# kfirc1503/generative-audio

Hardware: AMD Instinct MI355X
Metric: spectrogram-frames/sec, NPPC K=5 FullSubNet+ train step (higher is better)
Workload: dtype bf16

## Files before the change

### generative-audio_amd/csrc/tcn.hip

```cpp
#include <cstdlib>
#include "common.h"
#include "mfma_tile.h"
#include "nppc_hip.h"

namespace {


template <typename T, int EPI>
__global__ __launch_bounds__(256) void gemm_nt_kernel(GemmArgs g) {
  const int ks = g.ksplit > 1 ? g.ksplit : 1;
  const int z = blockIdx.z / ks, ksl = blockIdx.z % ks;
  const T* A = reinterpret_cast<const T*>(g.A) + (size_t)z * g.strideA + (size_t)ksl * g.K;
  const T* B = reinterpret_cast<const T*>(g.B) + (size_t)z * g.strideB + (size_t)ksl * g.K;
  const int lane = threadIdx.x & 63, wave = threadIdx.x >> 6, n = lane & 15, q = lane >> 4;
  const int r0 = blockIdx.x * 128 + wave * 32, c0 = blockIdx.y * 64;
  const T* ap = A + (size_t)(r0 + n) * g.lda + 8 * q;
  const T* bp = B + (size_t)(c0 + n) * g.ldb + 8 * q;
  f32x4 acc[2][4];
  nt_reg_mainloop<T>(acc, g.K / 32, g.lda, g.ldb, [&](int kk) { return ap + 32 * kk; }, [&](int kk) { return bp + 32 * kk; },
                     g.relu_in);

  const NtEpilogue<T, EPI> ep(g, z, blockIdx.x * 128);
  float s1 = 0.f, s2 = 0.f;
#pragma unroll
// ... 929 lines not shown
                     lda, (const bf16_t*)B1, ldb1, nt1, (const bf16_t*)B2, ldb2, N2, C, ldc, (long)M * ldc, R / ksplit, rowsum);
  NPPC_CHECK_LAUNCH();
  return NPPC_OK;
}

extern "C" int nppc_gemm_tn_splitk_batched(const void* A, long lda, long sA, const void* B, long ldb, long sB, float* C, long ldc,
                                           long sC, int M, int N, long R, int ksplit, int batch, void* stream) {
  if (batch < 1) return NPPC_EBADARG;
  return launch_tn(A, lda, B, ldb, C, ldc, M, N, R, ksplit, 1, 0, 0, stream, batch, sA, sB, sC);
}

extern "C" int nppc_gemm_tn_splitk_taps(const void* A, long lda, const void* B, long ldb, float* C, long ldc, int M, int N,
                                        long R, int ksplit, int Wp, int shift_a, void* stream) {
  return launch_tn(A, lda, B, ldb, C, ldc, M, N, R, ksplit, 9, Wp, shift_a, stream);
}
```

### generative-audio_amd/csrc/train_ops.hip

```cpp
#include "common.h"
#include "nppc_hip.h"

namespace {

template <typename T>
__global__ __launch_bounds__(256) void transpose_kernel(const T* __restrict__ in, T* __restrict__ out, int rows, int cols,
                                                        long ld_in, long ld_out, long sIn, long sOut, int relu) {
  __shared__ float tile[32][33];
  in += (size_t)blockIdx.z * sIn;
  out += (size_t)blockIdx.z * sOut;
  const int r0 = blockIdx.x * 32, c0 = blockIdx.y * 32;
  const int tx = threadIdx.x & 31, ty = threadIdx.x >> 5;
  for (int i = ty; i < 32; i += 8) {
    const int r = r0 + i, c = c0 + tx;
    float v = 0.f;
    if (r < rows && c < cols) v = to_f32<T>(in[(size_t)r * ld_in + c]);
    if (relu) v = fmaxf(v, 0.f);
    tile[i][tx] = v;
  }
  __syncthreads();
  for (int i = ty; i < 32; i += 8) {
    const int c = c0 + i, r = r0 + tx;
    if (c < cols && r < rows) out[(size_t)c * ld_out + r] = from_f32<T>(tile[tx][i]);
  }
// ... 326 lines not shown
  dst += (size_t)blockIdx.z * sDst;
  __shared__ float tile[32][33];
  const int c0 = blockIdx.x * 32, r0 = blockIdx.y * 32;
  const int tx = threadIdx.x & 31, ty = threadIdx.x >> 5;
  for (int i = ty; i < 32; i += 8) {
    const int c = c0 + i, r = r0 + tx;
    float a = 0.f;
    if (c < ncols && r < rows)
      for (int s = 0; s < S; ++s) a += slabs[(size_t)s * slab_stride + (size_t)c * ld + r];
    tile[i][tx] = a;
  }
  __syncthreads();
  for (int i = ty; i < 32; i += 8) {
    const int r = r0 + i, c = c0 + tx;
    if (r < rows && c < ncols) dst[(size_t)r * dst_ld + c] = tile[tx][i];
  }
}

__global__ void adam_kernel(float* __restrict__ p, const float* __restrict__ g, float* __restrict__ m, float* __restrict__ v,
                            long n, float lr, float b1, float b2, float eps, float wd, float bc1, float bc2_sqrt,
                            float gscale, const double* __restrict__ sumsq, float max_norm,
                            const unsigned* const* __restrict__ guards = nullptr, int n_guards = 0, float* poison = nullptr) {
  for (int i = 0; i < n_guards; ++i)
    if (*guards[i] != 0u) {
      if (poison && blockIdx.x == 0 && threadIdx.x == 0) *poison = __builtin_nanf("");
      return;
    }
  if (sumsq) {
    const float total = (float)sqrt(sumsq[0]) * gscale;
    const float coef = max_norm / (total + 1e-6f);
// ... 183 lines not shown
  hipLaunchKernelGGL(reduce_slabs_kernel, dim3(gx, 1, batch), dim3(256), 0, (hipStream_t)stream, slabs, S, slab_stride, ld,
                     dst, dst_ld, rows, col0, ncols, permH, accumulate, sSlab, sDst);
  NPPC_CHECK_LAUNCH();
  return NPPC_OK;
}

int nppc_reduce_slabs_t(const float* slabs, int S, long slab_stride, long ld, float* dst, long dst_ld, int rows, int ncols,
                        long sSlab, long sDst, int batch, void* stream) {
  if (!slabs || !dst || S < 1 || rows <= 0 || ncols <= 0 || batch < 1) return NPPC_EBADARG;
  hipLaunchKernelGGL(reduce_slabs_t_kernel, dim3(ceil_div(ncols, 32), ceil_div(rows, 32), batch), dim3(256), 0,
                     (hipStream_t)stream, slabs, S, slab_stride, ld, dst, dst_ld, rows, ncols, sSlab, sDst);
  NPPC_CHECK_LAUNCH();
  return NPPC_OK;
}

int nppc_adam_step(float* p, const float* g, float* m, float* v, long n, double lr, double b1, double b2, double eps,
                   double wd, int step, double gscale, void* stream) {
  if (!p || !g || !m || !v || n <= 0 || step < 1) return NPPC_EBADARG;
  const double bc1 = 1.0 - pow(b1, (double)step);
  const double bc2s = sqrt(1.0 - pow(b2, (double)step));
  const int grid = (int)((n + 255) / 256 > 2048 ? 2048 : (n + 255) / 256);
  hipLaunchKernelGGL(adam_kernel, dim3(grid), dim3(256), 0, (hipStream_t)stream, p, g, m, v, n, (float)lr, (float)b1, (float)b2,
                     (float)eps, (float)wd, (float)bc1, (float)bc2s, (float)gscale, (const double*)nullptr, 0.f);
  NPPC_CHECK_LAUNCH();
  return NPPC_OK;
}

int nppc_adam_step_guarded(float* p, const float* g, float* m, float* v, long n, double lr, double b1, double b2, double eps,
                           double wd, int step, double gscale, const void* guards, int n_guards, float* poison, void* stream) {
  if (!p || !g || !m || !v || n <= 0 || step < 1 || n_guards < 0 || (n_guards > 0 && !guards)) return NPPC_EBADARG;
// ... 24 lines not shown
```

### generative-audio_amd/nppc_audio/_hip.py

```python
import ctypes
import os
import threading

import torch

_HERE = os.path.dirname(os.path.abspath(__file__))
LIB_PATH = os.path.join(_HERE, "libnppc_hip.so")

PREC_BF16 = 0
PREC_F32 = 1
_ERR = {1: "bad argument", 2: "kernel launch failed", 3: "unsupported shape/configuration"}

_lib = None

c_p = ctypes.c_void_p
c_i = ctypes.c_int
c_l = ctypes.c_long
c_f = ctypes.c_float


def lib():
    global _lib
    if _lib is None:
        if not os.path.exists(LIB_PATH):
# ... 23 lines not shown
def check(rc, what):
    if rc != 0:
        raise RuntimeError(f"{what} failed: {_ERR.get(rc, rc)}")


def ptr_array(tensors):
    for t in tensors:
        assert t.is_cuda and t.is_contiguous()
    return (ctypes.c_void_p * len(tensors))(*[t.data_ptr() for t in tensors])


def mid_bwd_part_elems(B, C, Tp, batch):
    n = c_l()
    call("nppc_tcn_mid_bwd_part_elems", B, C, Tp, batch, ctypes.byref(n))
    return n.value


def conv_thin_part_elems():
    n = c_l()
    call("nppc_conv_thin_part_elems", ctypes.byref(n))
    return n.value


def masked_mse_work_elems():
    n = c_l()
    call("nppc_masked_mse_work_elems", ctypes.byref(n))
    return n.value


def crm_mse_work_elems():
# ... 51 lines not shown
                           I, I, I, I, I, I, P],
    "nppc_scale_transpose": [I, P, P, P, I, I, I, I, I, I, P],
    "nppc_gemm_nt": [I, I, P, L, L, P, L, L, P, L, L, P, L, P, L, L, P, L, P, L, I, I, I, I, I, I, I, I, I, P],
    "nppc_tcn_mid_bwd_part_elems": [I, I, I, I, PL],
    "nppc_tcn_mid_bwd": [I, P, P, P, P, P, P, P, P, P, P, P, P, P, P, P, P, P, P, P, P, P, P, P, P, P, P, I, I, I, P,
                         I, I, I, I, I, F, L, L, L, I, I, P],
    "nppc_tcn_mid_bwd_finish": [P, L, P, L, I, I, I, P, P, P, P, P, P, P, P, P, P, I, I, L, L, I, I, P],
    "nppc_gemm_nt_colsum": [I, I, P, L, L, P, L, L, P, L, L, P, L, P, L, L, I, I, I, I, I, I, I, P, P],
    "nppc_gemm_nt_gn": [I, P, L, L, P, L, L, P, L, L, P, P, L, P, L, L, P, L, D, F, I, I, I, I, I, I, I, P],
    "nppc_tcn_pack_sconv": [I, P, P, P, P, P, P, P, I, I, I, I, I, I, L, L, L, L, P],
    "nppc_gemm_nt_splitk": [I, P, L, P, L, P, L, I, I, L, I, P],
    "nppc_gemm_tn_splitk": [P, L, P, L, P, L, I, I, L, I, P],
    "nppc_gemm_tn_splitk_rowsum": [P, L, P, L, P, L, I, I, L, I, P, P],
    "nppc_gemm_tn_splitk2": [P, L, P, L, I, P, L, I, P, L, I, L, I, P, P],
    "nppc_gemm_tn_splitk_batched": [P, L, L, P, L, L, P, L, L, I, I, L, I, I, P],
    "nppc_reduce_slabs_t": [P, I, L, L, P, L, I, I, L, L, I, P],
    "nppc_gemm_tn_splitk_taps": [P, L, P, L, P, L, I, I, L, I, I, I, P],
    "nppc_tcn_dwconv": [I, P, P, P, P, P, P, P, P, P, I, I, I, I, I, I, F, L, L, L, I, P],
    "nppc_tcn_gn_apply": [I, P, P, P, P, P, I, I, I, I, I, F, L, L, L, I, P],
    "nppc_pack_matrix": [I, P, P, I, I, I, I, I, P],
    "nppc_pack_matrix_batched": [I, P, P, I, I, I, I, I, I, I, L, L, L, L, P],
    "nppc_subband_mean": [I, P, I, P, I, L, P, P, P, I, I, I, I, I, P],
    "nppc_subband_stage": [I, P, I, P, I, L, P, P, I, I, I, I, I, I, I, I, P],
    "nppc_sb_head": [I, P, P, P, P, L, I, I, I, I, I, P],
    "nppc_gram": [P, P, P, P, P, I, I, L, P],
    "nppc_combine": [P, P, P, P, P, P, P, I, I, L, P],
    "nppc_gs_solve": [P, P, P, I, I, I, P],
    "nppc_gs_bwd_solve": [P, P, P, P, I, I, I, P],
    "nppc_loss_solve": [P, P, P, P, P, P, P, P, P, P, I, I, P],
    "nppc_loss_bwd_coef": [P, P, P, F, F, P, I, I, P],
    "nppc_loss_bwd_coef_dev": [P, P, P, P, F, F, P, I, I, P],
    "nppc_transpose": [I, P, P, I, I, L, L, L, L, I, I, P],
    "nppc_colsum": [I, P, P, I, I, L, L, L, I, P, L, P],
    "nppc_colsum_scratch_elems": [I, I, I, PL],
    "nppc_sb_head_bwd": [I, P, P, P, P, P, P, L, I, I, I, I, I, P],
    "nppc_subband_stage_bwd": [I, P, P, P, P, P, P, I, I, I, I, I, L, I, I, I, P],
    "nppc_subband_unfold_bwd": [I, P, P, P, P, P, I, I, I, I, I, I, I, I, P],
    "nppc_reduce_slabs": [P, I, L, L, P, L, I, I, I, I, I, L, L, I, P],
    "nppc_adam_step": [P, P, P, P, L, D, D, D, D, D, I, D, P],
    "nppc_adam_step_guarded": [P, P, P, P, L, D, D, D, D, D, I, D, P, I, P, P],
    "nppc_loss_solve_eps": [P, P, P, P, P, P, P, P, P, P, I, I, D, I, P],
    "nppc_loss_solve_obj": [P, P, P, P, P, P, P, P, P, P, I, I, D, I, F, P, P],
    "nppc_mix_snr": [P, P, P, F, P, P, P, I, I, P],
    "nppc_inpaint_prepare": [P, P, P, I, F, P, P, P, I, I, I, I, I, P],
    "nppc_time_to_spec_mask": [P, P, I, I, I, I, I, I, P],
    "nppc_stft_pair": [P, P, P, P, I, I, I, I, P],
    "nppc_dropout": [I, P, L, L, I, F, L, I, P, P],
    "nppc_pca_work_elems": [I, I, I, PL],
    "nppc_pca_batch": [P, I, I, I, I, P, P, P, P, P, P, P],
    "nppc_pair_loss": [P, P, P, P, P, P, P, P, P, I, I, L, D, P],
    "nppc_pair_loss_bwd": [P, P, P, P, F, F, P, I, I, L, P],
    "nppc_metric_rows": [P, P, P, P, P, L, P],
    "nppc_rows_gram": [P, I, P, I, L, P, P],
# ... 153 lines not shown
```

### generative-audio_amd/nppc_audio/engine.py

```python
import ctypes

import numpy as np
import torch

from . import _hip as H
from .ops_lstm import (PackedLSTM, PackedLSTMBwd, ROW_PAD, WGRAD_SPLITS, bwd_head_fusable, forward_x_ld, lstm2_backward, lstm2_forward,
                       own_workspaces, padded_rows,
                       rows_view, workspace)

TCN_HIDDEN = 512
TCN_DILATIONS = (1, 2, 5, 9, 1, 2, 5, 9)
BRANCHES = ("", "_real", "_imag")
EPI_PLAIN, EPI_PRELU_STATS, EPI_RESIDUAL, EPI_RELU, EPI_PLAIN_F32, EPI_MASK_POS = 0, 1, 2, 3, 4, 5


def rup(a, b):
    return (a + b - 1) // b * b


TCN_WGRAD_SPLITS = 8
TCN_WGRAD_MAIN_BLOCKS = 1


class FlatParams:

    def __init__(self, module, device):
        named = list(module.named_parameters())
        total = sum(p.numel() for _, p in named)
        self.flat = torch.empty(total, dtype=torch.float32, device=device)
        self.grad = None
        self.off = {}
        o = 0
        for n, p in named:
            k = p.numel()
            self.flat[o:o + k].copy_(p.detach().reshape(-1))
            p.data = self.flat[o:o + k].view(p.shape)
# ... 371 lines not shown
                self.g(dest[3]).copy_(self.g(dest[2]))

        if self.prec == H.PREC_BF16 and K4 % 128 == 0 and Hd % 64 == 0 and KX % 64 == 0:
            S = WGRAD_SPLITS
            assert 64 * S <= ROW_PAD
            slab = ws("slab", (S * K4 * max(Hd, KX),), torch.float32)
            fold_bias = K4 % 256 == 0 and Hd % 128 == 0 and (K4 // 256) * (Hd // 128) * S >= 256
            if (guards is not None and fold_bias and Hd % 192 == 0 and KX == 64 and Tv > 1
                    and (K4 // 256) * (Hd // 192 + 1) * S >= 256):
                h1_guard, h2_guard = guards
                rows = (Rr + 64 * S - 1) // (64 * S) * (64 * S)
                slab = ws("slab2", (S * K4 * 2 * Hd,), torch.float32)
                rsum = ws("rowsum", (S, K4), torch.float32)
                H.call("nppc_gemm_tn_splitk2", dg1, K4, h1_guard, Hd, Hd, x_rows, KX, KX, slab, Hd + KX, K4, rows, S, None, s)
                n1 = K4 * (Hd + KX)
                H.call("nppc_reduce_slabs", slab, S, n1, Hd + KX, self.g(q + "weight_hh_l0"), Hd, K4, 0, Hd, Hd, 0, 0, 0, 1, s)
                H.call("nppc_reduce_slabs", slab, S, n1, Hd + KX, self.g(q + "weight_ih_l0"), I, K4, Hd, I, Hd, 0, 0, 0, 1, s)
                H.call("nppc_reduce_slabs", slab, S, n1, Hd + KX, self.g(q + "bias_ih_l0"), 1, K4, Hd + I, 1, Hd, 0, 0, 0, 1, s)
                self.g(q + "bias_hh_l0").copy_(self.g(q + "bias_ih_l0"))
                H.call("nppc_gemm_tn_splitk2", dg2, K4, h1_rows, Hd, Hd, h2_guard, Hd, Hd, slab, 2 * Hd, K4, rows, S, rsum, s)
                n2 = K4 * 2 * Hd
                H.call("nppc_reduce_slabs", slab, S, n2, 2 * Hd, self.g(q + "weight_ih_l1"), Hd, K4, 0, Hd, Hd, 0, 0, 0, 1, s)
                H.call("nppc_reduce_slabs", slab, S, n2, 2 * Hd, self.g(q + "weight_hh_l1"), Hd, K4, Hd, Hd, Hd, 0, 0, 0, 1, s)
                H.call("nppc_reduce_slabs", rsum, S, K4, 1, self.g(q + "bias_ih_l1"), 1, K4, 0, 1, Hd, 0, 0, 0, 1, s)
                self.g(q + "bias_hh_l1").copy_(self.g(q + "bias_ih_l1"))
                jobs = []
            for dg, off, inp, width, dest in jobs:
                rows = (Rr - off + 64 * S - 1) // (64 * S) * (64 * S)
                if fold_bias and dest[0] == "bias":
                    continue
                if fold_bias and dest == ("w", q + "weight_ih_l1"):
                    rsum = ws("rowsum", (S, K4), torch.float32)
                    H.call("nppc_gemm_tn_splitk_rowsum", dg.view(-1)[off * K4:], K4, inp, width, slab, width, K4, width, rows, S,
                           rsum, s)
                    H.call("nppc_reduce_slabs", rsum, S, K4, 1, self.g(q + "bias_ih_l1"), 1, K4, 0, 1, Hd, 0, 0, 0, 1, s)
                    self.g(q + "bias_hh_l1").copy_(self.g(q + "bias_ih_l1"))
                else:
                    H.call("nppc_gemm_tn_splitk", dg.view(-1)[off * K4:], K4, inp, width, slab, width, K4, width, rows, S, s)
                scatter(slab, S, K4, width, dest)
            if head is not None:
# ... 125 lines not shown
        h1b = ws("h1b", (3, B, Tp, TCN_HIDDEN))
        h2b = ws("h2b", (3, B, Tp, TCN_HIDDEN))
        Smid = ws("Smid", (3, B, TCN_HIDDEN // 64, 8), torch.float64)
        n_part = H.mid_bwd_part_elems(B, TCN_HIDDEN, Tp, 3)
        Pmid = ws("Pmid", (8, n_part), torch.float32)
        lay = self.fp.off["fb_model.sequence_model.1.conv1x1.weight"][0] - self.fp.off["fb_model.sequence_model.0.conv1x1.weight"][0]

        def finish_mid(lo, hi):
            pre_ = f"fb_model.sequence_model.{lo}."
            H.call("nppc_tcn_mid_bwd_finish", Pmid[lo], n_part, cpL[lo] if cs_ok else None, 3 * (R // 128) * ldC, R // 128, ldC, C,
                   self.g(pre_ + "norm2.weight"), self.g(pre_ + "norm2.bias"), self.g(pre_ + "norm1.weight"), self.g(pre_ + "norm1.bias"),
                   self.g(pre_ + "depthwise_conv.weight"), self.g(pre_ + "depthwise_conv.bias"), self.g(pre_ + "prelu1.weight"),
                   self.g(pre_ + "prelu2.weight"), self.g(pre_ + "conv1x1.bias"), self.g(pre_ + "sconv.bias") if cs_ok else None,
                   B, TCN_HIDDEN, sP, lay, 3, hi - lo, s)
        early = self.grad_range_hook is not None and self.early_buckets_ok
        dXo, dXi = dXa, dXb
        for i in range(7, -1, -1):
            pre = f"fb_model.sequence_model.{i}."
            dil = TCN_DILATIONS[i]
            st1, st2 = d["stats"][i, 0], d["stats"][i, 1]
            y1, y2, Xin = d["y1"][i], d["y2"][i], d["X"][i]
            if tn_ok:
                dXo, dXi, a2, h2b = dXL[i + 1], dXL[i], a2L[i], h2L[i]
            else:
                a2 = d["a2"]
            if not cs_ok:
                H.colsum(prec, dXo, self.g(pre + "sconv.bias"), R, C, ldC, R * ldC, sP, 3,
                         lambda n: ws("cs_sconv", (n,), torch.float32), s)
            H.call("nppc_gemm_nt", prec, EPI_PLAIN, dXo, ldC, R * ldC, self.W2T[i], ldC, TCN_HIDDEN * ldC, h1b, TCN_HIDDEN,
                   sAct, None, 0, None, 0, 0, None, 0, None, 0, R, TCN_HIDDEN, ldC, Tp, Tv, TCN_HIDDEN, 0, 3, 1, s)
            H.call("nppc_tcn_mid_bwd", prec, h1b, y2, y1, st1, st2, Smid, Pmid[i], self.p(pre + "norm1.weight"), self.p(pre + "norm1.bias"),
                   self.p(pre + "norm2.weight"), self.p(pre + "norm2.bias"), self.p(pre + "depthwise_conv.weight"),
                   self.p(pre + "prelu1.weight"), self.p(pre + "prelu2.weight"), a2, h2b, self.g(pre + "norm2.weight"),
                   self.g(pre + "norm2.bias"), self.g(pre + "norm1.weight"), self.g(pre + "norm1.bias"),
                   self.g(pre + "depthwise_conv.weight"), self.g(pre + "depthwise_conv.bias"), self.g(pre + "prelu1.weight"),
                   self.g(pre + "prelu2.weight"), self.g(pre + "conv1x1.bias"),
                   cpL[i] if cs_ok else None, R // 128, ldC, C, self.g(pre + "sconv.bias") if cs_ok else None,
                   B, TCN_HIDDEN, Tp, Tv, dil, 1e-8, sAct, B * 2, sP, 3, 0, s)
            if i == 4 and early:
                finish_mid(4, 8)
            if tn_ok:
                inline = i < TCN_WGRAD_MAIN_BLOCKS
                wslab = ws("slab_main", (3 * S2 * TCN_HIDDEN * ldC,), torch.float32) if inline else slab2

                def sconv_wgrad(a2=a2, dXo=dXo, dest=self.g(pre + "sconv.weight"), wslab=wslab):
                    q = H.stream()
                    H.call("nppc_gemm_tn_splitk_batched", a2, TCN_HIDDEN, sAct, dXo, ldC, R * ldC, wslab, ldC,
                           S2 * TCN_HIDDEN * ldC, TCN_HIDDEN, ldC, R, S2, 3, q)
                    H.call("nppc_reduce_slabs_t", wslab, S2, TCN_HIDDEN * ldC, ldC, dest, TCN_HIDDEN, C, TCN_HIDDEN,
                           S2 * TCN_HIDDEN * ldC, sP, 3, q)
                if inline:
                    sconv_wgrad()
                else:
                    on_side(sconv_wgrad)
            else:
                H.call("nppc_transpose", prec, dXo, tA, R, ldC, ldC, R, R * ldC, sTA, 0, 3, s)
                H.call("nppc_transpose", prec, a2, tB, R, TCN_HIDDEN, TCN_HIDDEN, R, sAct, sTB, 0, 3, s)
                self._wgrad(tA, R, sTA, tB, R, sTB, Cr, TCN_HIDDEN, R, S2, pre + "sconv.weight", TCN_HIDDEN, C, TCN_HIDDEN,
                            slab2, batch=3, sDst=sP)
            if tn_ok:
                def c1_wgrad(h2b=h2b, Xin=Xin, dest=self.g(pre + "conv1x1.weight"), wslab=wslab):
                    q = H.stream()
                    H.call("nppc_gemm_tn_splitk_batched", h2b, TCN_HIDDEN, sAct, Xin, ldC, R * ldC, wslab, ldC,
                           S2 * TCN_HIDDEN * ldC, TCN_HIDDEN, ldC, R, S2, 3, q)
                    H.call("nppc_reduce_slabs", wslab, S2, TCN_HIDDEN * ldC, ldC, dest, C, TCN_HIDDEN, 0, C, 0, 0,
                           S2 * TCN_HIDDEN * ldC, sP, 3, q)
                if inline:
                    c1_wgrad()
                else:
                    on_side(c1_wgrad)
            else:
                H.call("nppc_transpose", prec, h2b, tA, R, TCN_HIDDEN, TCN_HIDDEN, R, sAct, sTA, 0, 3, s)
                H.call("nppc_transpose", prec, Xin, tB, R, ldC, ldC, R, R * ldC, sTB, 0, 3, s)
                self._wgrad(tA, R, sTA, tB, R, sTB, TCN_HIDDEN, ldC, R, S2, pre + "conv1x1.weight", C, TCN_HIDDEN, C, slab2,
                            batch=3, sDst=sP)
# ... 10 lines not shown
                        a = self.fp.off[f"fb_model{br}.sequence_model.4.conv1x1.weight"][0]
                        b, shp = self.fp.off[f"fb_model{br}.sequence_model.7.sconv.bias"]
                        self.grad_range_hook(G, a, b + int(np.prod(shp)))
                on_side(blocks_done)
        finish_mid(0, 4 if early else 8)
        if tn_ok:
            dXo = dXL[0]
        if self.nm == 1:
            H.call("nppc_subband_unfold_bwd", prec, dx, d["sbscale"], Dsb, self.mult, dXo[0], ldC, B, F, Tp, Tv, self.nb, self.G,
                   self.KX, s)
        sv = d["tsse_saved"]
        n_ws = ctypes.c_long()
        H.call("nppc_tsse_bwd_ws_elems", 3 * self.nm, B, F, self.ks[0], self.ks[1], self.ks[2], ctypes.byref(n_ws))
        dsg = ws("dsg", (n_ws.value,), torch.float32)
        att = "channel_attention."
        H.call("nppc_tsse_bwd_maps", prec, dXo, R * ldC, H.ptr_array(d["maps"]), 3 * self.nm, d["rs"],
               self.p(att + "smallConv1d.0.weight"), self.p(att + "middleConv1d.0.weight"), self.p(att + "largeConv1d.0.weight"),
               self.ks[0], self.ks[1], self.ks[2], self.p(att + "feature_concate_fc.weight"), self.p(att + "fc1.weight"),
               self.p(att + "fc2.weight"), self.sAtt, sv["ns"], sv["pre"], sv["sq"], sv["h1"], sv["sg"], dsg,
               self.g(att + "smallConv1d.0.weight"), self.g(att + "smallConv1d.0.bias"),
               self.g(att + "middleConv1d.0.weight"), self.g(att + "middleConv1d.0.bias"),
               self.g(att + "largeConv1d.0.weight"), self.g(att + "largeConv1d.0.bias"),
               self.g(att + "feature_concate_fc.weight"), self.g(att + "feature_concate_fc.bias"),
               self.g(att + "fc1.weight"), self.g(att + "fc1.bias"), self.g(att + "fc2.weight"), self.g(att + "fc2.bias"),
               B, F, T, self.la, Tp, ldC, s)
        if tn_ok:
            fc_wgrad(ws("slab_fc", (3 * S2 * Fr * ldC,), torch.float32))
        if self.defer_join:
            self.join_pending = True
            FSNEngine._unjoined[id(self)] = self
        else:
            torch.cuda.current_stream().wait_stream(self._side)
        return G

    def side_stream(self):
        return self._side

    def prepack_on_side(self):
        ev = torch.cuda.Event()
        ev.record(torch.cuda.current_stream())
# ... 17 lines not shown
```

### include/nppc_hip.h

```cpp
#ifndef NPPC_HIP_H
#define NPPC_HIP_H
#ifdef __cplusplus
extern "C" {
#endif

int nppc_stft(const float* wave, float* re, float* im, float* mag , int B, int L, int nfft, int hop,
              void* stream);
int nppc_dropband(const float* in, float* out, int B, int C, int F, int T, int G, void* stream);
int nppc_cirm_build_compress(const float* nr, const float* ni, const float* cr, const float* ci, float* out, int B, int F,
                             int T, int G, float eps, void* stream);
int nppc_cirm_decompress_apply_conj(const float* crm, const float* nr, const float* ni, float* dec ,
                                    float* emag, float* ere, float* eim, int B, int F, int T, void* stream);

int nppc_cirm_decompress_apply(const float* crm, const float* nr, const float* ni, float* dec , float* emag,
                               float* ere, float* eim, int B, int F, int T, void* stream);
int nppc_istft(const float* re, const float* im, float* out, int B, int T, int nfft, int hop, int L, void* stream);

int nppc_rowsum(const float* x, double* sums, long R, int T, void* stream);
int nppc_tsse_fwd_maps(int prec, const float* const* maps, int nmaps, double* rowsum, const float* cw0, const float* cb0,
                       const float* cw1, const float* cb1, const float* cw2, const float* cb2, int ks0, int ks1, int ks2,
                       const float* fcw, const float* fcb, const float* w1, const float* b1, const float* w2, const float* b2, long sW,
                       float* scale, float* ns, float* pre, float* sq, float* h1, float* sg, void* X0, long sY, int B, int C, int T,
                       int look_ahead, int Tp, int ld, void* stream);
int nppc_tsse_bwd_ws_elems(int nmaps, int B, int C, int ks0, int ks1, int ks2, long* elems);
// ... 21 lines not shown
                 long sC, const float* bias, long sBias, const void* res, long ldres, long sRes, const float* slope,
                 long sSlope, double* stats, long sStats, int R, int N, int K, int Tp, int Tv, int Nv, int relu_in,
                 int batch, int ksplit, void* stream);
int nppc_gemm_nt_splitk(int prec, const void* A, long lda, const void* B, long ldb, float* C, long ldc, int M, int N, long K,
                        int ksplit, void* stream);
int nppc_gemm_tn_splitk(const void* A, long lda, const void* B, long ldb, float* C, long ldc, int M, int N, long R, int ksplit,
                        void* stream);
int nppc_gemm_tn_splitk_rowsum(const void* A, long lda, const void* B, long ldb, float* C, long ldc, int M, int N, long R,
                               int ksplit, float* rowsum, void* stream);
int nppc_gemm_tn_splitk2(const void* A, long lda, const void* B1, long ldb1, int N1, const void* B2, long ldb2, int N2, float* C,
                         long ldc, int M, long R, int ksplit, float* rowsum, void* stream);
int nppc_gemm_tn_splitk_batched(const void* A, long lda, long sA, const void* B, long ldb, long sB, float* C, long ldc, long sC,
                                int M, int N, long R, int ksplit, int batch, void* stream);
int nppc_gemm_tn_splitk_taps(const void* A, long lda, const void* B, long ldb, float* C, long ldc, int M, int N, long R,
                             int ksplit, int Wp, int shift_a, void* stream);
int nppc_pack_matrix(int prec, const float* src, void* dst, int N, int K, int Npad, int ldd, int transpose, void* stream);
int nppc_pack_matrix_batched(int prec, const float* src, void* dst, int N, int K, int Npad, int ldd, int transpose, int n_a,
                             int n_b, long src_stride_a, long src_stride_b, long dst_stride_a, long dst_stride_b, void* stream);
int nppc_tcn_dwconv(int prec, const void* in, void* out, const double* st1, double* st2, const float* gamma,
                    const float* beta, const float* wd, const float* bd, const float* slope2, int B, int Cc, int ld, int Tp,
                    int Tv, int dil, float eps, long sAct, long sSt, long sP, int batch, void* stream);
int nppc_tcn_gn_apply(int prec, const void* in, void* out, const double* st, const float* gamma, const float* beta, int B,
                      int Cc, int ld, int Tp, int Tv, float eps, long sAct, long sSt, long sP, int batch, void* stream);
int nppc_tcn_gn_bwd(int prec, const void* dA, const void* y, const double* st, const float* gamma, const float* slope,
                    double* S, void* dpre, float* dgamma, float* dbeta, float* dslope, int B, int Cc, int Tp, int Tv, float eps,
                    long sAct, long sSt, long sP, int batch, void* stream);
int nppc_tcn_dwconv_bwd(int prec, const void* du, const void* y1, const double* st1, const float* gamma, const float* beta,
                        const float* wd, void* dz, float* dwd, float* dbd, int B, int Cc, int Tp, int Tv, int dil, float eps,
                        long sAct, long sSt, long sP, int batch, void* stream);
int nppc_tcn_mid_bwd_part_elems(int B, int Cc, int Tp, int batch, long* n);
// ... 15 lines not shown
int nppc_gemm_nt_colsum(int prec, int epi, const void* A, long lda, long sA, const void* B, long ldb, long sB, void* C, long ldc,
                        long sC, const float* bias, long sBias, const void* res, long ldres, long sRes, int R, int N, int K,
                        int Tp, int Tv, int Nv, int batch, float* colpart, void* stream);
int nppc_tcn_pack_sconv(int prec, const float* W, const float* gamma, const float* beta, const float* bias, void* Wg, float* u,
                        float* v, int N, int K, int Npad, int ldd, int n_a, int n_b, long src_stride_a, long src_stride_b,
                        long dst_stride_a, long dst_stride_b, void* stream);
int nppc_transpose(int prec, const void* in, void* out, int rows, int cols, long ld_in, long ld_out, long sIn, long sOut,
                   int relu, int batch, void* stream);
int nppc_colsum_scratch_elems(int rows, int cols, int batch, long* n);
int nppc_colsum(int prec, const void* M, float* out, int rows, int cols, long ld, long sM, long sOut, int batch,
                float* scratch, long scratch_elems, void* stream);
int nppc_reduce_slabs_t(const float* slabs, int S, long slab_stride, long ld, float* dst, long dst_ld, int rows, int ncols,
                        long sSlab, long sDst, int batch, void* stream);
int nppc_reduce_slabs(const float* slabs, int S, long slab_stride, long ld, float* dst, long dst_ld, int rows, int col0,
                      int ncols, int permH, int accumulate, long sSlab, long sDst, int batch, void* stream);

int nppc_subband_mean(int prec, const void* src, int ldS, const void* fb, int ldF, long strideFb, const float* mult,
                      float* scale, double* work, int B, int F, int Tp, int Tv, int nfeat, void* stream);
int nppc_subband_stage(int prec, const void* src, int ldS, const void* fb, int ldF, long strideFb, const float* scale,
                       void* x, int B, int F, int Tp, int Tv, int nb, int G, int KX, int ones_col, void* stream);
int nppc_subband_stage_bwd(int prec, const void* dx, const void* x, const void* fb, const float* scale, double* D,
                           void* dpre, int B, int F, int Tp, int Tv, int ldF, long strideFb, int nb, int G, int KX,
                           void* stream);
int nppc_subband_unfold_bwd(int prec, const void* dx, const float* scale, const double* D, const float* mult, void* dX0,
                            int ldX, int B, int F, int Tp, int Tv, int nb, int G, int KX, void* stream);
int nppc_sb_head(int prec, const void* h2, const void* wh, const float* bias, float* out, long Nseq, int Tn, int la,
                 int Hd, int O, int Fo, void* stream);
int nppc_sb_head_bwd(int prec, const float* dout, const void* whT, const void* h2, void* dh2, float* dWh, float* dbh,
                     long Nseq, int Tn, int la, int Hd, int O, int Fo, void* stream);

// ... 372 lines not shown
```

Measured before the change: 251,600.

## Group TCN block weight-grads into one persistent split-K launch with fused finish

Adds a grouped kernel that computes all six TCN block weight-gradient GEMMs (three depthwise-sconv and three conv1x1 branches) in one launch, with a planner that picks the split-K factor to fill the CUs. A fused finish kernel reduces the slabs and writes transposed or direct outputs. This replaces the separate transpose, batched GEMM and reduce launches. LSTM weight-grad slab reductions and bias copies are merged into one finish kernel, and the TSSE backward is moved onto the side stream. The aim is fewer launches and better CU occupancy, at the cost of more workspace and more side-stream contention.

```diff
diff --git a/generative-audio_amd/csrc/tcn.hip b/generative-audio_amd/csrc/tcn.hip
--- a/generative-audio_amd/csrc/tcn.hip
+++ b/generative-audio_amd/csrc/tcn.hip
@@ -967,3 +967,162 @@
                                         long R, int ksplit, int Wp, int shift_a, void* stream) {
   return launch_tn(A, lda, B, ldb, C, ldc, M, N, R, ksplit, 9, Wp, shift_a, stream);
 }
+
+namespace {
+
+constexpr int WG_MAXP = 8;
+constexpr int WG_BN = 192, WG_BR = 32, WG_STAGES = 5;
+constexpr int WG_SMEM = WG_STAGES * (WG_BR * DR_BM * 2 + WG_BR * WG_BN * 2);
+
+struct WgradTable {
+  const bf16_t* A[WG_MAXP];
+  const bf16_t* B[WG_MAXP];
+  float* slab[WG_MAXP];
+};
+
+__global__ __launch_bounds__(512, 1) void tcn_wgrad_block_kernel(WgradTable t, long lda, long ldb, long ldc, long slab_stride,
+                                                                 int mt, int nt, int S, long nstage) {
+  const unsigned W = gridDim.x, lin = blockIdx.x;
+  const unsigned x = lin & 7, j = lin >> 3, q = W >> 3, rem = W & 7;
+  const unsigned work = x * q + (x < rem ? x : rem) + j;
+  const unsigned tiles = (unsigned)(mt * nt);
+  const unsigned grp = work / tiles, tt = work % tiles;
+  const unsigned p = grp / (unsigned)S, z = grp % (unsigned)S;
+  const unsigned bx = tt % (unsigned)mt, by = tt / (unsigned)mt;
+  const long s_lo = (long)z * nstage / S, s_hi = (long)(z + 1) * nstage / S;
+  const long rbase = s_lo * WG_BR;
+  dma_tile<DR_BM, WG_BN, WG_BR, WG_STAGES>(t.A[p], lda, t.B[p], ldb, t.slab[p] + (size_t)z * slab_stride, ldc, (long)bx * DR_BM,
+                                          (long)by * WG_BN, (long)by * WG_BN, rbase, rbase, (s_hi - s_lo) * WG_BR, nullptr);
+}
+
+struct WgradFinTable {
+  const float* slab[WG_MAXP];
+  float* dst[WG_MAXP];
+  int transposed[WG_MAXP];
+};
+
+__global__ __launch_bounds__(256) void tcn_wgrad_finish_kernel(WgradFinTable t, int S, long slab_stride, long ldc, int M, int C) {
+  __shared__ float tile[64][65];
+  const int p = blockIdx.z;
+  const float* __restrict__ sl = t.slab[p];
+  float* __restrict__ dst = t.dst[p];
+  const bool tr = t.transposed[p] != 0;
+  const int c0 = blockIdx.x * 64, m0 = blockIdx.y * 64;
+  const int tid = threadIdx.x, cq = tid & 15, mr = tid >> 4;
+#pragma unroll
+  for (int pass = 0; pass < 4; ++pass) {
+    const int m = mr + 16 * pass;
+    const float* src = sl + (size_t)(m0 + m) * ldc + c0 + 4 * cq;
+    float4 a = {0.f, 0.f, 0.f, 0.f};
+#pragma unroll 4
+    for (int s = 0; s < S; ++s) {
+      const float4 v = *reinterpret_cast<const float4*>(src + (size_t)s * slab_stride);
+      a.x += v.x;
+      a.y += v.y;
+      a.z += v.z;
+      a.w += v.w;
+    }
+    if (tr) {
+      tile[m][4 * cq + 0] = a.x;
+      tile[m][4 * cq + 1] = a.y;
+      tile[m][4 * cq + 2] = a.z;
+      tile[m][4 * cq + 3] = a.w;
+    } else {
+      float* d = dst + (size_t)(m0 + m) * C;
+      const int c = c0 + 4 * cq;
+      if (c + 0 < C) d[c + 0] = a.x;
+      if (c + 1 < C) d[c + 1] = a.y;
+      if (c + 2 < C) d[c + 2] = a.z;
+      if (c + 3 < C) d[c + 3] = a.w;
+    }
+  }
+  if (!tr) return;
+  __syncthreads();
+  const int m = tid & 63;
+  for (int c = tid >> 6; c < 64; c += 4)
+    if (c0 + c < C) dst[(size_t)(c0 + c) * M + m0 + m] = tile[m][c];
+}
+
+int wgrad_block_plan(int nprob, int M, int N, long R, int n_cu, int S_req, int* S_out, int* wg_out, int* ncu_out) {
+  if (nprob < 1 || nprob > WG_MAXP || M <= 0 || N <= 0 || R <= 0) return NPPC_EBADARG;
+  if (M % DR_BM || N % WG_BN || R % WG_BR) return NPPC_EUNSUPPORTED;
+  if (n_cu <= 0) {
+    int dev = 0;
+    if (hipGetDevice(&dev) != hipSuccess ||
+        hipDeviceGetAttribute(&n_cu, hipDeviceAttributeMultiprocessorCount, dev) != hipSuccess || n_cu <= 0)
+      return NPPC_ELAUNCH;
+  }
+  const long tiles = (long)nprob * (M / DR_BM) * (N / WG_BN), n = R / WG_BR;
+  long S = 0;
+  if (S_req > 0) {
+    S = S_req < n ? S_req : n;
+  } else {
+    double best = -1.0;
+    for (int k = 1; k <= 16; ++k) {
+      long s = (long)k * n_cu / tiles;
+      if (s < 1) continue;
+      if (s > n) s = n;
+      const double fill = (double)(tiles * s - (long)(k - 1) * n_cu) / n_cu;
+      if (fill > best) {
+        best = fill;
+        S = s;
+      }
+      if (fill >= 0.9 || s == n) break;
+    }
+    if (S < 1) S = 1;
+  }
+  if (tiles * S > 0x7fffffffL) return NPPC_EUNSUPPORTED;
+  if (S_out) *S_out = (int)S;
+  if (wg_out) *wg_out = (int)(tiles * S);
+  if (ncu_out) *ncu_out = n_cu;
+  return NPPC_OK;
+}
+
+}
+
+extern "C" int nppc_tcn_wgrad_block_plan(int nprob, int M, int N, long R, int n_cu, int S_req, int* S, int* workgroups, int* n_cu_used) {
+  return wgrad_block_plan(nprob, M, N, R, n_cu, S_req, S, workgroups, n_cu_used);
+}
+
+extern "C" int nppc_tcn_wgrad_block(const void* const* A, long lda, const void* const* B, long ldb, float* const* slab, long ldc,
+                                    int nprob, int M, int N, long R, int S, void* stream) {
+  if (!A || !B || !slab) return NPPC_EBADARG;
+  int wg = 0;
+  const int rc = wgrad_block_plan(nprob, M, N, R, 0, S, &S, &wg, nullptr);
+  if (rc != NPPC_OK) return rc;
+  if (lda < M || ldb < N || ldc < N) return NPPC_EBADARG;
+  if (lda % 8 || ldb % 8) return NPPC_EUNSUPPORTED;
+  WgradTable t = {};
+  for (int p = 0; p < nprob; ++p) {
+    if (!A[p] || !B[p] || !slab[p]) return NPPC_EBADARG;
+    if ((size_t)A[p] % 16 || (size_t)B[p] % 16) return NPPC_EUNSUPPORTED;
+    t.A[p] = (const bf16_t*)A[p];
+    t.B[p] = (const bf16_t*)B[p];
+    t.slab[p] = slab[p];
+  }
+  if (hipFuncSetAttribute(reinterpret_cast<const void*>(tcn_wgrad_block_kernel), hipFuncAttributeMaxDynamicSharedMemorySize,
+                          WG_SMEM) != hipSuccess)
+    return NPPC_ELAUNCH;
+  hipLaunchKernelGGL(tcn_wgrad_block_kernel, dim3(wg), dim3(512), WG_SMEM, (hipStream_t)stream, t, lda, ldb, ldc, (long)M * ldc,
+                     M / DR_BM, N / WG_BN, S, R / WG_BR);
+  NPPC_CHECK_LAUNCH();
+  return NPPC_OK;
+}
+
+extern "C" int nppc_tcn_wgrad_block_finish(const float* const* slab, float* const* dst, const int* transposed, int nprob, int S,
+                                           int M, long ldc, int C, void* stream) {
+  if (!slab || !dst || !transposed || nprob < 1 || nprob > WG_MAXP || S < 1 || M <= 0 || C <= 0 || ldc < C) return NPPC_EBADARG;
+  if (M % 64 || ldc % 64) return NPPC_EUNSUPPORTED;
+  WgradFinTable t = {};
+  for (int p = 0; p < nprob; ++p) {
+    if (!slab[p] || !dst[p]) return NPPC_EBADARG;
+    if ((size_t)slab[p] % 16) return NPPC_EUNSUPPORTED;
+    t.slab[p] = slab[p];
+    t.dst[p] = dst[p];
+    t.transposed[p] = transposed[p];
+  }
+  hipLaunchKernelGGL(tcn_wgrad_finish_kernel, dim3((C + 63) / 64, M / 64, nprob), dim3(256), 0, (hipStream_t)stream, t, S,
+                     (long)M * ldc, ldc, M, C);
+  NPPC_CHECK_LAUNCH();
+  return NPPC_OK;
+}
diff --git a/generative-audio_amd/csrc/train_ops.hip b/generative-audio_amd/csrc/train_ops.hip
--- a/generative-audio_amd/csrc/train_ops.hip
+++ b/generative-audio_amd/csrc/train_ops.hip
@@ -364,6 +364,57 @@
   for (int i = ty; i < 32; i += 8) {
     const int r = r0 + i, c = c0 + tx;
     if (r < rows && c < ncols) dst[(size_t)r * dst_ld + c] = tile[tx][i];
+  }
+}
+
+struct LstmFinArgs {
+  const float* slab;
+  const float* rsum;
+  float *dstA, *dstB, *bias1, *bias2;
+  long slab_stride, ld;
+  int S, rows, permH, colA, ncolA, colB, ncolB, bias_col;
+};
+
+__global__ __launch_bounds__(256) void lstm_wgrad_finish_kernel(LstmFinArgs a) {
+  const int qpr = (int)(a.ld >> 2);
+  const long nq = (long)a.rows * qpr, total = nq + (a.rsum ? a.rows : 0);
+  for (long e = (long)blockIdx.x * blockDim.x + threadIdx.x; e < total; e += (long)gridDim.x * blockDim.x) {
+    const int r = e < nq ? (int)(e / qpr) : (int)(e - nq);
+    int rr = r;
+    if (a.permH > 0) {
+      const int u = r >> 2, gp = r & 3;
+      const int tg = gp == 0 ? 0 : (gp == 1 ? 2 : (gp == 2 ? 1 : 3));
+      rr = tg * a.permH + u;
+    }
+    if (e >= nq) {
+      float s = 0.f;
+      for (int k = 0; k < a.S; ++k) s += a.rsum[(size_t)k * a.rows + r];
+      a.bias1[rr] = s;
+      a.bias2[rr] = s;
+      continue;
+    }
+    const int c0 = 4 * (int)(e % qpr);
+    const float* src = a.slab + (size_t)r * a.ld + c0;
+    float4 v = {0.f, 0.f, 0.f, 0.f};
+#pragma unroll 8
+    for (int k = 0; k < a.S; ++k) {
+      const float4 w = *reinterpret_cast<const float4*>(src + (size_t)k * a.slab_stride);
+      v.x += w.x;
+      v.y += w.y;
+      v.z += w.z;
+      v.w += w.w;
+    }
+    const float vv[4] = {v.x, v.y, v.z, v.w};
+#pragma unroll
+    for (int i = 0; i < 4; ++i) {
+      const int c = c0 + i;
+      if (c >= a.colA && c < a.colA + a.ncolA) a.dstA[(size_t)rr * a.ncolA + (c - a.colA)] = vv[i];
+      else if (c >= a.colB && c < a.colB + a.ncolB) a.dstB[(size_t)rr * a.ncolB + (c - a.colB)] = vv[i];
+      else if (c == a.bias_col) {
+        a.bias1[rr] = vv[i];
+        a.bias2[rr] = vv[i];
+      }
+    }
   }
 }
 
@@ -577,6 +628,24 @@
   return NPPC_OK;
 }
 
+int nppc_lstm_wgrad_finish(const float* slab, int S, long slab_stride, long ld, int rows, int permH, float* dstA, int colA,
+                           int ncolA, float* dstB, int colB, int ncolB, int bias_col, const float* rsum, float* bias1,
+                           float* bias2, void* stream) {
+  if (!slab || !dstA || S < 1 || rows <= 0 || ld <= 0 || colA < 0 || ncolA <= 0 || colA + ncolA > ld) return NPPC_EBADARG;
+  if (dstB ? (colB < 0 || ncolB <= 0 || colB + ncolB > ld) : ncolB != 0) return NPPC_EBADARG;
+  if (dstB && colB < colA + ncolA && colA < colB + ncolB) return NPPC_EBADARG;
+  if ((bias_col >= 0 || rsum) && (!bias1 || !bias2)) return NPPC_EBADARG;
+  if (bias_col >= ld || (bias_col >= 0 && rsum)) return NPPC_EBADARG;
+  if (permH > 0 && rows != 4 * permH) return NPPC_EBADARG;
+  if (ld % 4 || slab_stride % 4 || (size_t)slab % 16) return NPPC_EUNSUPPORTED;
+  LstmFinArgs a = {slab, rsum, dstA, dstB, bias1, bias2, slab_stride, ld, S, rows, permH, colA, ncolA, colB, ncolB, bias_col};
+  const long total = (long)rows * (ld / 4) + (rsum ? rows : 0);
+  const int gx = (int)((total + 255) / 256 > 4096 ? 4096 : (total + 255) / 256);
+  hipLaunchKernelGGL(lstm_wgrad_finish_kernel, dim3(gx), dim3(256), 0, (hipStream_t)stream, a);
+  NPPC_CHECK_LAUNCH();
+  return NPPC_OK;
+}
+
 int nppc_adam_step(float* p, const float* g, float* m, float* v, long n, double lr, double b1, double b2, double eps,
                    double wd, int step, double gscale, void* stream) {
   if (!p || !g || !m || !v || n <= 0 || step < 1) return NPPC_EBADARG;
diff --git a/generative-audio_amd/nppc_audio/_hip.py b/generative-audio_amd/nppc_audio/_hip.py
--- a/generative-audio_amd/nppc_audio/_hip.py
+++ b/generative-audio_amd/nppc_audio/_hip.py
@@ -61,6 +61,19 @@
     n = c_l()
     call("nppc_tcn_mid_bwd_part_elems", B, C, Tp, batch, ctypes.byref(n))
     return n.value
+
+
+def tcn_wgrad_block_plan(nprob, M, N, R, S_req=0, n_cu=0):
+    S, wg, cu = c_i(), c_i(), c_i()
+    rc = _bind("nppc_tcn_wgrad_block_plan")(nprob, M, N, R, n_cu, S_req, ctypes.byref(S), ctypes.byref(wg), ctypes.byref(cu))
+    if rc == 3:
+        return None
+    check(rc, "nppc_tcn_wgrad_block_plan")
+    return S.value, wg.value, cu.value
+
+
+def addr_array(addrs):
+    return (ctypes.c_void_p * len(addrs))(*addrs)
 
 
 def conv_thin_part_elems():
@@ -142,6 +155,9 @@
     "nppc_gemm_tn_splitk_rowsum": [P, L, P, L, P, L, I, I, L, I, P, P],
     "nppc_gemm_tn_splitk2": [P, L, P, L, I, P, L, I, P, L, I, L, I, P, P],
     "nppc_gemm_tn_splitk_batched": [P, L, L, P, L, L, P, L, L, I, I, L, I, I, P],
+    "nppc_tcn_wgrad_block_plan": [I, I, I, L, I, I, PI, PI, PI],
+    "nppc_tcn_wgrad_block": [P, L, P, L, P, L, I, I, I, L, I, P],
+    "nppc_tcn_wgrad_block_finish": [P, P, P, I, I, I, L, I, P],
     "nppc_reduce_slabs_t": [P, I, L, L, P, L, I, I, L, L, I, P],
     "nppc_gemm_tn_splitk_taps": [P, L, P, L, P, L, I, I, L, I, I, I, P],
     "nppc_tcn_dwconv": [I, P, P, P, P, P, P, P, P, P, I, I, I, I, I, I, F, L, L, L, I, P],
@@ -165,6 +181,7 @@
     "nppc_subband_stage_bwd": [I, P, P, P, P, P, P, I, I, I, I, I, L, I, I, I, P],
     "nppc_subband_unfold_bwd": [I, P, P, P, P, P, I, I, I, I, I, I, I, I, P],
     "nppc_reduce_slabs": [P, I, L, L, P, L, I, I, I, I, I, L, L, I, P],
+    "nppc_lstm_wgrad_finish": [P, I, L, L, I, I, P, I, I, P, I, I, I, P, P, P, P],
     "nppc_adam_step": [P, P, P, P, L, D, D, D, D, D, I, D, P],
     "nppc_adam_step_guarded": [P, P, P, P, L, D, D, D, D, D, I, D, P, I, P, P],
     "nppc_loss_solve_eps": [P, P, P, P, P, P, P, P, P, P, I, I, D, I, P],
diff --git a/generative-audio_amd/nppc_audio/engine.py b/generative-audio_amd/nppc_audio/engine.py
--- a/generative-audio_amd/nppc_audio/engine.py
+++ b/generative-audio_amd/nppc_audio/engine.py
@@ -20,6 +20,7 @@
 
 TCN_WGRAD_SPLITS = 8
 TCN_WGRAD_MAIN_BLOCKS = 1
+TCN_WGRAD_BLOCK_MAIN_BLOCKS = 0
 
 
 class FlatParams:
@@ -421,16 +422,12 @@
                 rsum = ws("rowsum", (S, K4), torch.float32)
                 H.call("nppc_gemm_tn_splitk2", dg1, K4, h1_guard, Hd, Hd, x_rows, KX, KX, slab, Hd + KX, K4, rows, S, None, s)
                 n1 = K4 * (Hd + KX)
-                H.call("nppc_reduce_slabs", slab, S, n1, Hd + KX, self.g(q + "weight_hh_l0"), Hd, K4, 0, Hd, Hd, 0, 0, 0, 1, s)
-                H.call("nppc_reduce_slabs", slab, S, n1, Hd + KX, self.g(q + "weight_ih_l0"), I, K4, Hd, I, Hd, 0, 0, 0, 1, s)
-                H.call("nppc_reduce_slabs", slab, S, n1, Hd + KX, self.g(q + "bias_ih_l0"), 1, K4, Hd + I, 1, Hd, 0, 0, 0, 1, s)
-                self.g(q + "bias_hh_l0").copy_(self.g(q + "bias_ih_l0"))
+                H.call("nppc_lstm_wgrad_finish", slab, S, n1, Hd + KX, K4, Hd, self.g(q + "weight_hh_l0"), 0, Hd,
+                       self.g(q + "weight_ih_l0"), Hd, I, Hd + I, None, self.g(q + "bias_ih_l0"), self.g(q + "bias_hh_l0"), s)
                 H.call("nppc_gemm_tn_splitk2", dg2, K4, h1_rows, Hd, Hd, h2_guard, Hd, Hd, slab, 2 * Hd, K4, rows, S, rsum, s)
                 n2 = K4 * 2 * Hd
-                H.call("nppc_reduce_slabs", slab, S, n2, 2 * Hd, self.g(q + "weight_ih_l1"), Hd, K4, 0, Hd, Hd, 0, 0, 0, 1, s)
-                H.call("nppc_reduce_slabs", slab, S, n2, 2 * Hd, self.g(q + "weight_hh_l1"), Hd, K4, Hd, Hd, Hd, 0, 0, 0, 1, s)
-                H.call("nppc_reduce_slabs", rsum, S, K4, 1, self.g(q + "bias_ih_l1"), 1, K4, 0, 1, Hd, 0, 0, 0, 1, s)
-                self.g(q + "bias_hh_l1").copy_(self.g(q + "bias_ih_l1"))
+                H.call("nppc_lstm_wgrad_finish", slab, S, n2, 2 * Hd, K4, Hd, self.g(q + "weight_ih_l1"), 0, Hd,
+                       self.g(q + "weight_hh_l1"), Hd, Hd, -1, rsum, self.g(q + "bias_ih_l1"), self.g(q + "bias_hh_l1"), s)
                 jobs = []
             for dg, off, inp, width, dest in jobs:
                 rows = (Rr - off + 64 * S - 1) // (64 * S) * (64 * S)
@@ -586,6 +583,11 @@
                    self.g(pre_ + "prelu2.weight"), self.g(pre_ + "conv1x1.bias"), self.g(pre_ + "sconv.bias") if cs_ok else None,
                    B, TCN_HIDDEN, sP, lay, 3, hi - lo, s)
         early = self.grad_range_hook is not None and self.early_buckets_ok
+        blk = H.tcn_wgrad_block_plan(6, TCN_HIDDEN, ldC, R) if tn_ok else None
+        if blk is not None:
+            blk_sl = blk[0] * TCN_HIDDEN * ldC
+            blk_slab = ws("slab_blk", (6 * blk_sl,), torch.float32)
+            blk_tr = (ctypes.c_int * 6)(1, 1, 1, 0, 0, 0)
         dXo, dXi = dXa, dXb
         for i in range(7, -1, -1):
             pre = f"fb_model.sequence_model.{i}."
@@ -611,7 +613,25 @@
                    B, TCN_HIDDEN, Tp, Tv, dil, 1e-8, sAct, B * 2, sP, 3, 0, s)
             if i == 4 and early:
                 finish_mid(4, 8)
-            if tn_ok:
+            if blk is not None:
+                inline = i < TCN_WGRAD_BLOCK_MAIN_BLOCKS
+                wslab = ws("slab_blk_main", (6 * blk_sl,), torch.float32) if inline else blk_slab
+
+                def block_wgrad(a2=a2, dXo=dXo, h2b=h2b, Xin=Xin, d2=self.g(pre + "sconv.weight"),
+                                d1=self.g(pre + "conv1x1.weight"), wslab=wslab):
+                    q = H.stream()
+                    br = range(3)
+                    A = H.addr_array([a2.data_ptr() + 2 * z * sAct for z in br] + [h2b.data_ptr() + 2 * z * sAct for z in br])
+                    Bm = H.addr_array([dXo.data_ptr() + 2 * z * R * ldC for z in br] + [Xin.data_ptr() + 2 * z * R * ldC for z in br])
+                    sl = H.addr_array([wslab.data_ptr() + 4 * j * blk_sl for j in range(6)])
+                    dst = H.addr_array([d2.data_ptr() + 4 * z * sP for z in br] + [d1.data_ptr() + 4 * z * sP for z in br])
+                    H.call("nppc_tcn_wgrad_block", A, TCN_HIDDEN, Bm, ldC, sl, ldC, 6, TCN_HIDDEN, ldC, R, blk[0], q)
+                    H.call("nppc_tcn_wgrad_block_finish", sl, dst, blk_tr, 6, blk[0], TCN_HIDDEN, ldC, C, q)
+                if inline:
+                    block_wgrad()
+                else:
+                    on_side(block_wgrad)
+            elif tn_ok:
                 inline = i < TCN_WGRAD_MAIN_BLOCKS
                 wslab = ws("slab_main", (3 * S2 * TCN_HIDDEN * ldC,), torch.float32) if inline else slab2
 
@@ -630,7 +650,9 @@
                 H.call("nppc_transpose", prec, a2, tB, R, TCN_HIDDEN, TCN_HIDDEN, R, sAct, sTB, 0, 3, s)
                 self._wgrad(tA, R, sTA, tB, R, sTB, Cr, TCN_HIDDEN, R, S2, pre + "sconv.weight", TCN_HIDDEN, C, TCN_HIDDEN,
                             slab2, batch=3, sDst=sP)
-            if tn_ok:
+            if blk is not None:
+                pass
+            elif tn_ok:
                 def c1_wgrad(h2b=h2b, Xin=Xin, dest=self.g(pre + "conv1x1.weight"), wslab=wslab):
                     q = H.stream()
                     H.call("nppc_gemm_tn_splitk_batched", h2b, TCN_HIDDEN, sAct, Xin, ldC, R * ldC, wslab, ldC,
@@ -671,16 +693,22 @@
         H.call("nppc_tsse_bwd_ws_elems", 3 * self.nm, B, F, self.ks[0], self.ks[1], self.ks[2], ctypes.byref(n_ws))
         dsg = ws("dsg", (n_ws.value,), torch.float32)
         att = "channel_attention."
-        H.call("nppc_tsse_bwd_maps", prec, dXo, R * ldC, H.ptr_array(d["maps"]), 3 * self.nm, d["rs"],
-               self.p(att + "smallConv1d.0.weight"), self.p(att + "middleConv1d.0.weight"), self.p(att + "largeConv1d.0.weight"),
-               self.ks[0], self.ks[1], self.ks[2], self.p(att + "feature_concate_fc.weight"), self.p(att + "fc1.weight"),
-               self.p(att + "fc2.weight"), self.sAtt, sv["ns"], sv["pre"], sv["sq"], sv["h1"], sv["sg"], dsg,
-               self.g(att + "smallConv1d.0.weight"), self.g(att + "smallConv1d.0.bias"),
-               self.g(att + "middleConv1d.0.weight"), self.g(att + "middleConv1d.0.bias"),
-               self.g(att + "largeConv1d.0.weight"), self.g(att + "largeConv1d.0.bias"),
-               self.g(att + "feature_concate_fc.weight"), self.g(att + "feature_concate_fc.bias"),
-               self.g(att + "fc1.weight"), self.g(att + "fc1.bias"), self.g(att + "fc2.weight"), self.g(att + "fc2.bias"),
-               B, F, T, self.la, Tp, ldC, s)
+
+        def tsse_bwd(dXo=dXo):
+            H.call("nppc_tsse_bwd_maps", prec, dXo, R * ldC, H.ptr_array(d["maps"]), 3 * self.nm, d["rs"],
+                   self.p(att + "smallConv1d.0.weight"), self.p(att + "middleConv1d.0.weight"), self.p(att + "largeConv1d.0.weight"),
+                   self.ks[0], self.ks[1], self.ks[2], self.p(att + "feature_concate_fc.weight"), self.p(att + "fc1.weight"),
+                   self.p(att + "fc2.weight"), self.sAtt, sv["ns"], sv["pre"], sv["sq"], sv["h1"], sv["sg"], dsg,
+                   self.g(att + "smallConv1d.0.weight"), self.g(att + "smallConv1d.0.bias"),
+                   self.g(att + "middleConv1d.0.weight"), self.g(att + "middleConv1d.0.bias"),
+                   self.g(att + "largeConv1d.0.weight"), self.g(att + "largeConv1d.0.bias"),
+                   self.g(att + "feature_concate_fc.weight"), self.g(att + "feature_concate_fc.bias"),
+                   self.g(att + "fc1.weight"), self.g(att + "fc1.bias"), self.g(att + "fc2.weight"), self.g(att + "fc2.bias"),
+                   B, F, T, self.la, Tp, ldC, H.stream())
+        if blk is not None:
+            on_side(tsse_bwd)
+        else:
+            tsse_bwd()
         if tn_ok:
             fc_wgrad(ws("slab_fc", (3 * S2 * Fr * ldC,), torch.float32))
         if self.defer_join:
diff --git a/include/nppc_hip.h b/include/nppc_hip.h
--- a/include/nppc_hip.h
+++ b/include/nppc_hip.h
@@ -59,6 +59,11 @@
                                 int M, int N, long R, int ksplit, int batch, void* stream);
 int nppc_gemm_tn_splitk_taps(const void* A, long lda, const void* B, long ldb, float* C, long ldc, int M, int N, long R,
                              int ksplit, int Wp, int shift_a, void* stream);
+int nppc_tcn_wgrad_block_plan(int nprob, int M, int N, long R, int n_cu, int S_req, int* S, int* workgroups, int* n_cu_used);
+int nppc_tcn_wgrad_block(const void* const* A, long lda, const void* const* B, long ldb, float* const* slab, long ldc, int nprob,
+                         int M, int N, long R, int S, void* stream);
+int nppc_tcn_wgrad_block_finish(const float* const* slab, float* const* dst, const int* transposed, int nprob, int S, int M,
+                                long ldc, int C, void* stream);
 int nppc_pack_matrix(int prec, const float* src, void* dst, int N, int K, int Npad, int ldd, int transpose, void* stream);
 int nppc_pack_matrix_batched(int prec, const float* src, void* dst, int N, int K, int Npad, int ldd, int transpose, int n_a,
                              int n_b, long src_stride_a, long src_stride_b, long dst_stride_a, long dst_stride_b, void* stream);
@@ -104,6 +109,9 @@
                         long sSlab, long sDst, int batch, void* stream);
 int nppc_reduce_slabs(const float* slabs, int S, long slab_stride, long ld, float* dst, long dst_ld, int rows, int col0,
                       int ncols, int permH, int accumulate, long sSlab, long sDst, int batch, void* stream);
+int nppc_lstm_wgrad_finish(const float* slab, int S, long slab_stride, long ld, int rows, int permH, float* dstA, int colA,
+                           int ncolA, float* dstB, int colB, int ncolB, int bias_col, const float* rsum, float* bias1,
+                           float* bias2, void* stream);
 
 int nppc_subband_mean(int prec, const void* src, int ldS, const void* fb, int ldF, long strideFb, const float* mult,
                       float* scale, double* work, int B, int F, int Tp, int Tv, int nfeat, void* stream);
```

After: 251,000. No clear change (-0.3%).
